# estebandito22/Amplifai-DeepContentRecommenders

Hardware: AMD Instinct MI355X
Metric: training triplets/sec (whole node) + AUC@val, DCUE d=128 at 1/2/4/8 MI355X (higher is better)
Workload: dtype f32 (conv forwards, input and weight gradients: f32 values as power-of-two-scaled split fp16 hi+lo pairs on f16 MFMA, f32 accumulate)

## Files before the change

### amplifai-deepcontentrecommenders_amd/csrc/adam.hip

```cpp
#include <mutex>
#include <unordered_map>

#include "dcue_internal.h"
#include "tgemm.h"
#include "bn0adam.h"


DCUE_KTRACE_READER(adam)

namespace dcue {

__device__ __forceinline__ bool idle_moments(float m, float v) {
  return (__float_as_uint(m) | __float_as_uint(v)) == 0u;
}
__device__ __forceinline__ bool idle_moments4(const float4& m, const float4& v) {
  return (__float_as_uint(m.x) | __float_as_uint(m.y) | __float_as_uint(m.z) | __float_as_uint(m.w) |
          __float_as_uint(v.x) | __float_as_uint(v.y) | __float_as_uint(v.z) | __float_as_uint(v.w)) == 0u;
}
__device__ __forceinline__ float wave_max(float x) {
#pragma unroll
  for (int o = 32; o > 0; o >>= 1) x = fmaxf(x, __shfl_xor(x, o));
  return x;
}
__device__ __forceinline__ float wave_min(float x) {
// ... 718 lines not shown
  sc.one_m_b2 = (float)(1.0 - a->beta2);
  sc.bc2_sqrt = (float)pow(bc2, 0.5);
  sc.eps = (float)a->eps;
  sc.wd = (float)a->weight_decay;
  sc.inv_bc2_sqrt = 1.0f / sc.bc2_sqrt;
  return sc;
}


__global__ __launch_bounds__(256) void k_bn0_grads_adam(const float* __restrict__ G, const float* __restrict__ E,
                                                        const float* gamma0, const float* beta0, const float* mean0,
                                                        const float* invstd0, int H, float* dgamma0, float* dbeta0,
                                                        Bn0AdamDev a) {
  critical_path_priority();
  __shared__ float rg[256], rb[256];
  bn0_channel<true>(G, E, gamma0, beta0, mean0, invstd0, H, dgamma0, dbeta0, a, nullptr, nullptr, nullptr,
                    blockIdx.x, threadIdx.x, rg, rb, true);
}

Bn0AdamDev bn0adam_dev(const Bn0Adam& a) {
  const dcue_model* md = a.md;
  Bn0AdamDev d;
  d.p = md->params; d.m = md->exp_avg; d.v = md->exp_avg_sq; d.g = md->grads;
  d.o_w1 = a.poff[seg_conv_w(1)]; d.o_cb1 = a.poff[seg_conv_b(1)];
  d.o_g0 = a.bn ? a.poff[seg_bn_w(0)] : -1; d.o_b0 = a.bn ? a.poff[seg_bn_b(0)] : -1;
  d.o_g1 = a.bn ? a.poff[seg_bn_w(1)] : -1; d.o_b1 = a.bn ? a.poff[seg_bn_b(1)] : -1;
  d.sc = form_scalars(&a.args);
  d.seg1 = pack_args(md, a.poff).seg[0];
  d.wpack = md->wpack;
  return d;
}

int launch_bn0_grads_adam(const float* G, const float* E, const float* gamma0, const float* beta0,
                          const float* mean0, const float* invstd0, int H, float* dgamma0, float* dbeta0,
                          const Bn0Adam& a, hipStream_t s) {
  const dcue_model* md = a.md;
  if (H > 256) return DCUE_ERR_UNSUPPORTED;
  if (!md->params || !md->grads || !md->exp_avg || !md->exp_avg_sq || a.args.grad_div > 1.0) return DCUE_ERR_INVALID;
  const Bn0AdamDev d = bn0adam_dev(a);
  DCUE_LAUNCH(k_bn0_grads_adam, dim3(kMels), dim3(256), 0, s, G, E, gamma0, beta0, mean0, invstd0, H, dgamma0,
              dbeta0, d);
  DCUE_LAUNCH_CHECK();
  return DCUE_OK;
}

long adam_dense_blocks(long len) { return len >= 512L * 1024 ? 512 : (len / 4 + 255) / 256 + 1; }

int launch_adam(const dcue_model* md, const dcue_adam_args* a, const int64_t* poff, hipStream_t s,
                bool flush_slice, long dense_lo, long dense_hi, bool defer_dgrad2, unsigned* sig) {
  const AdamScalars sc = form_scalars(a);
  const float gdiv = a->grad_div > 1.0 ? (float)a->grad_div : 0.f;
  const int parts = a->parts ? a->parts : (DCUE_ADAM_DENSE | DCUE_ADAM_EMBEDDING);
  const long n = dense_hi >= 0 ? dense_hi : poff[DCUE_N_DENSE_SEGMENTS];
  if (parts & DCUE_ADAM_DENSE) {
    const long len = n - dense_lo;
    const long blocks = adam_dense_blocks(len);
// ... 74 lines not shown
```

### amplifai-deepcontentrecommenders_amd/csrc/bn0adam.h

```cpp
#pragma once

#include "dcue_internal.h"

namespace dcue {

#define DCUE_RHD __device__ __forceinline__
DCUE_RHD float rn_fma(float a, float b, float c) { return __fmaf_rn(a, b, c); }
DCUE_RHD float rn_mul(float a, float b) { return __fmul_rn(a, b); }
DCUE_RHD float rn_add(float a, float b) { return __fadd_rn(a, b); }
DCUE_RHD float rn_sub(float a, float b) { return __fsub_rn(a, b); }
DCUE_RHD float rn_div(float a, float b) { return __fdiv_rn(a, b); }
DCUE_RHD float rn_sqrt(float a) { return __builtin_sqrtf(a); }

}

#include "adam_replay.h"

namespace dcue {

struct Bn0AdamDev {
  float *p, *m, *v, *g;
  long o_w1, o_cb1, o_g0, o_b0, o_g1, o_b1;
  AdamScalars sc;
  PackSeg seg1;
  float* wpack;
};

__device__ __forceinline__ void adam_at(const Bn0AdamDev& a, long idx, float gr) {
  float pp = a.p[idx], mm = a.m[idx], vv = a.v[idx];
  adam_elem(pp, gr, mm, vv, a.sc);
  a.p[idx] = pp;
  a.m[idx] = mm;
  a.v[idx] = vv;
}
Bn0AdamDev bn0adam_dev(const Bn0Adam& a);

template <bool ADAM>
DCUE_RHD void bn0_channel(const float* __restrict__ G, const float* __restrict__ E, const float* gamma0,
                          const float* beta0, const float* mean0, const float* invstd0, int H, float* dgamma0,
                          float* dbeta0, const Bn0AdamDev& a, const float* __restrict__ W1, float* dW1, float* db1,
                          int c, int t, float* rg, float* rb, bool active) {
  float* __restrict__ P = a.p;
  float* __restrict__ Mo = a.m;
  float* __restrict__ V = a.v;
  float* __restrict__ Gd = a.g;
  float dg = 0.f, db = 0.f;
  float pg = 0.f, mg = 0.f, vg = 0.f, pb = 0.f, mb = 0.f, vb = 0.f;
  if (active) {
    if (ADAM && t == 0 && a.o_g0 >= 0) {
      pg = P[a.o_g0 + c]; mg = Mo[a.o_g0 + c]; vg = V[a.o_g0 + c];
      pb = P[a.o_b0 + c]; mb = Mo[a.o_b0 + c]; vb = V[a.o_b0 + c];
    }
    const Bn0Chan ch = bn0_chan(gamma0, beta0, mean0, invstd0, c);
    constexpr int kMaxIt = 4;
#pragma unroll
    for (int it = 0; it < kMaxIt; ++it) {
      const int e = t + 256 * it;
      if (e < 4 * H) {
        const int o = e >> 2, k = e & 3;
        const long wi = ((long)o * kMels + c) * 4 + k;
        if constexpr (ADAM) {
          const long idx = a.o_w1 + wi;
          float pp = P[idx];
          const float gw = bn0_elem(G, E, H, ch, o, k, c, pp, dg, db);
          Gd[idx] = gw;
          float mm = Mo[idx], vv = V[idx];
          adam_elem(pp, gw, mm, vv, a.sc);
          P[idx] = pp;
          Mo[idx] = mm;
          V[idx] = vv;
          pack_store(a.seg1, wi, pp, a.wpack);
        } else {
          dW1[wi] = bn0_elem(G, E, H, ch, o, k, c, W1[wi], dg, db);
        }
      }
    }
    if constexpr (ADAM) {
      if (c == 0)
        for (int o = t; o < H; o += 256) {
          a.g[a.o_cb1 + o] = E[o];
          adam_at(a, a.o_cb1 + o, E[o]);
        }
      if (c == 1 && a.o_g1 >= 0)
        for (int o = t; o < H; o += 256) {
          adam_at(a, a.o_g1 + o, a.g[a.o_g1 + o]);
          adam_at(a, a.o_b1 + o, a.g[a.o_b1 + o]);
        }
    } else {
      if (c == 0)
        for (int o = t; o < H; o += 256) db1[o] = E[o];
    }
  }
  rg[t] = dg;
  rb[t] = db;
  __syncthreads();
  for (int off = 128; off > 0; off >>= 1) {
    if (t < off) {
      rg[t] += rg[t + off];
      rb[t] += rb[t + off];
    }
    __syncthreads();
  }
  if (active && t == 0) {
    dgamma0[c] = rg[0];
    dbeta0[c] = rb[0];
    if (ADAM && a.o_g0 >= 0) {
      adam_elem(pg, rg[0], mg, vg, a.sc);
      adam_elem(pb, rb[0], mb, vb, a.sc);
      P[a.o_g0 + c] = pg; Mo[a.o_g0 + c] = mg; V[a.o_g0 + c] = vg;
      P[a.o_b0 + c] = pb; Mo[a.o_b0 + c] = mb; V[a.o_b0 + c] = vb;
    }
  }
}

}
```

### amplifai-deepcontentrecommenders_amd/csrc/capi.hip

```cpp
#include <math.h>
#include <atomic>
#include <functional>
#include <string.h>

#include "dcue_internal.h"

using namespace dcue;

namespace dcue {

unsigned sync_event_flags() {
  static const unsigned f = [] {
    const char* e = getenv("DCUE_EVENT_SCOPE");
    return (e && e[0] == 's') ? (unsigned)hipEventDisableTiming
                              : (unsigned)(hipEventDisableTiming | hipEventReleaseToDevice);
  }();
  return f;
}

SidePool* side_pool() {
  static SidePool pools[64];
  int dev = 0;
  if (hipGetDevice(&dev) != hipSuccess || dev < 0 || dev >= 64) return nullptr;
  SidePool& p = pools[dev];
// ... 1395 lines not shown
    wa.x_a = l == 1 ? w.invstd[0] : w.a[l - 1];
    wa.x_beta = l == 1 ? nullptr : c.beta_bwd(w, l - 1);
    wa.g_l = w.g[l]; wa.y_l = w.y[l]; wa.idx_l = w.idx[l];
    wa.mean_l = w.mean[l]; wa.invstd_l = w.invstd[l]; wa.a_l = w.a[l];
    wa.dz_acc = bn_acc(w.bnbacc, w.cmax, l); wa.dgamma = c.dgamma(w, l); wa.dbeta = c.dbeta(w, l);
    wa.invN = c.bn ? (float)(1.0 / (copies * gm.lp)) : 0.f;
    wa.bn_world = bn_world;
    wa.counts = w.counts;
    wa.M = M; wa.cout = C; wa.cin = cin;
    wa.wpart = w.wpart[ps]; wa.bpart = w.bpart[ps];
    if (f16w) {
      wa.x_range = rng_at(w, l - 1); wa.y_range = rng_at(w, l); wa.g_range = grng_at(w, l);
      wa.kd_max = kd_max * wa.invN;
    }
    if (l == 1 && inputs_dev) wa.wait = o.inputs_wait;
    const int nch = wgrad_nchunk(l, M, C, cin);
    if (l == 1 && !f16w) {
      TRY(launch_conv1_dx(wa, w.dx1, so));
      wa.g_l = w.dx1;
    }
    TimerScope tsc;
    TRY(timer_begin(&tsc, l == 1 ? DCUE_TIMED_CONV1_WGRAD : -1, so));
    HPROF("capi:19");
    TRY(launch_conv_wgrad(l, l == 1 ? src : SRC_ACT, wa, nch, so));
    HPROF("capi:20");
    TRY(timer_end(&tsc));
    HPROF("capi:21");
    if (l != 1) {
      ForkAfter fk(sp, so, tail);
      TRY(launch_wgrad_reduce(l, wa.wpart, wa.bpart, nch, C, cin, c.Gd(seg_conv_w(l)),
                              c.Gd(seg_conv_b(l)), w.G, w.S, so));
      return fk.done();
    }
    TRY(launch_wgrad_reduce(l, wa.wpart, wa.bpart, nch, C, cin, c.Gd(seg_conv_w(l)),
                            c.Gd(seg_conv_b(l)), w.G, w.S, so));
    ForkAfter fk(sp, so, tail);
    const bool graw = f16w && src == SRC_TRACK_F16;
    if (fuse_late) {
      Bn0Adam ba;
      ba.md = m; ba.poff = c.poff; ba.args = *o.dense_split; ba.bn = c.bn;
      TRY(launch_bn0_grads_adam(w.G, w.S, c.gamma(w, 0), c.beta(w, 0), graw ? w.mean[0] : nullptr,
                                graw ? w.invstd[0] : nullptr, H, c.dgamma(w, 0), c.dbeta(w, 0), ba, so));
      TRY(fk.done());
      if (!probes_on()) return DCUE_OK;
      TRY(probe(PR_G_1, m->grads, late, so));
      return probe(PR_P_EARLY, m->params, late, so);
    }
    TRY(launch_bn0_grads(w.G, w.S, c.P(seg_conv_w(1)), c.gamma(w, 0), c.beta(w, 0),
                         graw ? w.mean[0] : nullptr, graw ? w.invstd[0] : nullptr, H,
                         c.Gd(seg_conv_w(1)), c.dgamma(w, 0), c.dbeta(w, 0),
                         c.Gd(seg_conv_b(1)), so));
    TRY(fk.done());
    return probe(PR_G_1, m->grads, late, so);
  };
  if (ev_x0) TRY(wait_point(s, ev_x0));
  if (o.wait_inputs && !inputs_via_late) {
    TRY(side.wait(o.ahead ? ahead_seq : o.wait_inputs_seq));
    if (!inputs_dev) TRY(wait_point(s, o.wait_inputs));
  }
  TRY(debug_delay(DCUE_SITE_WGRAD_1, s));
  TRY(issue_wgrad(1, s, 2, o.dense_split && !o.comm ? nullptr : &tail[0]));
  HPROF("capi:22");

  if (!thr) {
    if (c.res || c.text) TRY(fc_text_wgrad());
    if (fork_once()) ev_layer[3] = ev_layer[2];
// ... 140 lines not shown
```

### amplifai-deepcontentrecommenders_amd/csrc/conv_wgrad.hip

```cpp
#include "dcue_internal.h"
#include "bn0adam.h"

namespace dcue {

DCUE_KTRACE_READER(wgrad)
static constexpr int kWgradRch = 72;

template <int SRCX, int KS, int PAD, int LIN, int R, int POOL, int LP, int RCH, bool EDGES, bool RAW = false>
__device__ __forceinline__ void wgrad_body(const WgradArgs& a, int bx, int by, int bz, float* lds) {
  constexpr int PW = 128 + 16;
  constexpr int NB = EDGES ? 5 : 1;
  constexpr int FR = RCH / 8;
  constexpr bool TRACK = SRCX == SRC_TRACK_F16 || SRCX == SRC_TRACK_F32;
  float* dzs = lds;
  float* xs = lds + RCH * PW;
  float (*bsum)[NB][128] = reinterpret_cast<float (*)[NB][128]>(lds + 2 * RCH * PW);

  const int tid = threadIdx.x, lane = tid & 63, wave = tid >> 6;
  const int g = lane >> 4, l16 = lane & 15;
  const int wo = wave >> 1, wk = wave & 1;
  const int cout = a.cout, cin = a.cin, kcn = KS * cin;
  const int obase = by * 128, kcbase = bx * 128;
  const long total = (long)a.M * R;
  const long r_begin = (long)bz * a.rows_per_chunk;
// ... 634 lines not shown

constexpr int kW16tO = 64;
constexpr int kW16tThreads = 512;
constexpr int kWgItems = 128;
template <int R, int KS>
constexpr int w16t_img_rows() { return kW16Rows + (KS - 1) * (R >= kW16Rows ? 2 : kW16Rows / R + 2); }
template <int R, int KS>
constexpr size_t w16t_lds_bytes(bool xraw) {
  const size_t st = (size_t)2 * kW16Rows * 128 + (size_t)(xraw ? 1 : 2) * w16t_img_rows<R, KS>() * 256 +
                    (size_t)(kW16tO + 128 + 2 * kWgItems) * sizeof(int);
  const size_t ep = (size_t)kW16tO * (KS * 128 + 4) * sizeof(float);
  return st > ep ? st : ep;
}
__device__ __forceinline__ int w16_off128(int r, int ch) { return 128 * r + 16 * (ch ^ ((r & 2) | ((r >> 1) & 4))); }

template <int SRCX, int KS, int PAD, int LIN, int R, int POOL, int LP>
__device__ __forceinline__ void wgrad16t_body(const WgradArgs& a, int by, int bz, char* lds) {
  constexpr int RCH = kW16Rows;
  constexpr bool TRACK = SRCX == SRC_TRACK_F16 || SRCX == SRC_TRACK_F32;
  constexpr bool EDGES = TRACK;
  constexpr int NB = EDGES ? 5 : 1;
  constexpr int HALO = KS - 1;
  constexpr int IMG = w16t_img_rows<R, KS>();
  constexpr int FX = (IMG + 15) / 16;
  static_assert(KS == 4 && POOL == 4 && R % POOL == 0, "8 waves = 4 taps x 2 o halves; 16 windows per stage");
  constexpr bool TWO = R >= RCH;
  constexpr bool XRAW = SRCX == SRC_TRACK_F16;
  static_assert(TRACK || SRCX == SRC_ACT, "x: the track table (layer 1) or y_{l-1}");
  char* dzh = lds;
  char* dzl = dzh + RCH * 128;
  char* xh = dzl + RCH * 128;
  char* xl = xh + IMG * 256;
  int* exp_o = reinterpret_cast<int*>(xh + (XRAW ? 1 : 2) * IMG * 256);
// ... 280 lines not shown

  DCUE_KT(KID, 3);
  int eo_bias;
  {
    constexpr int KC = KS * 128, PITCH = KC + 4;
    int eo_r[2][4], ec_r[8];
#pragma unroll
    for (int m = 0; m < 2; ++m)
#pragma unroll
      for (int j = 0; j < 4; ++j) eo_r[m][j] = exp_o[32 * oh + 16 * m + 4 * g + j];
#pragma unroll
    for (int n = 0; n < 8; ++n) ec_r[n] = exp_c[16 * n + l16];
    eo_bias = tid < kW16tO ? exp_o[tid] : 0;
    __syncthreads();
    float* tl = reinterpret_cast<float*>(lds);
#pragma unroll
    for (int n = 0; n < 8; ++n)
#pragma unroll
      for (int m = 0; m < 2; ++m)
#pragma unroll
        for (int j = 0; j < 4; ++j)
          tl[(32 * oh + 16 * m + 4 * g + j) * PITCH + kx * 128 + 16 * n + l16] =
              ldexpf(acc[m][n][j], -(eo_r[m][j] + ec_r[n]));
    __syncthreads();
    const int nrow = min(kW16tO, cout - obase);
    float* wp = a.wpart + ((size_t)bz * cout + obase) * KC;
    constexpr int Q = KC / 4;
    for (int i = tid; i < nrow * Q; i += kW16tThreads) {
      const int r = i / Q, k4 = i - r * Q;
      st4(wp + (size_t)r * KC + 4 * k4, *reinterpret_cast<const float4*>(tl + r * PITCH + 4 * k4));
    }
    __syncthreads();
  }
  if (dzt)
#pragma unroll
    for (int e = 0; e < NB; ++e) st4(&bsum[ws][e][4 * q], bacc[e]);
  __syncthreads();
  if (tid < kW16tO && obase + tid < cout) {
#pragma unroll
    for (int e = 0; e < NB; ++e) {
      float v = 0.f;
#pragma unroll
      for (int sl = 0; sl < 16; ++sl) v += bsum[sl][e][tid];
      a.bpart[((size_t)bz * NB + e) * cout + obase + tid] = ldexpf(v, -eo_bias);
    }
  }
  DCUE_KT(KID, 4);
  DCUE_KTW(KID, 7);
}

template <int SRCX, int KS, int PAD, int LIN, int R, int POOL, int LP>
__global__ __launch_bounds__(kW16tThreads, 1) void k_conv_wgrad16t(WgradArgs a) {
  if constexpr (SRCX != SRC_ACT) critical_path_priority();
  extern __shared__ __attribute__((aligned(16))) char lds16t[];
  const int ot = (a.cout + kW16tO - 1) / kW16tO;
  const int L = xcd_swizzle(blockIdx.x, gridDim.x);
  wgrad16t_body<SRCX, KS, PAD, LIN, R, POOL, LP>(a, L % ot, L / ot, lds16t);
  if constexpr (SRCX != SRC_ACT) dev_wait_order(a.wait);
}

constexpr int kW1kO = 32;
constexpr int kW1kThreads = 256;
template <int R, int KS>
constexpr size_t w1k_lds_bytes() {
  const size_t st = (size_t)2 * kW16Rows * 128 + (size_t)w16t_img_rows<R, KS>() * 256 + kW1kO * sizeof(int) +
                    (size_t)kWgItems * (sizeof(int) + sizeof(float));
  const size_t ep = (size_t)kW1kO * (128 + 4) * sizeof(float);
  const size_t bs = (size_t)16 * 5 * kW1kO * sizeof(float);
  const size_t m = st > ep ? st : ep;
  return m > bs ? m : bs;
}

// ... 667 lines not shown
  if (wgrad_f16_on() && !bound)
    n = (rows + w16_rows_per_chunk(rows, (int)n) - 1) / w16_rows_per_chunk(rows, (int)n);
  return (int)(n < 1 ? 1 : n);
}

int wgrad_kernel(int layer, int cin, int cout, int src, bool alone) {
  if (layer == 1) {
    if (!wgrad_f16_on()) return WK_CONV1;
    if (src == SRC_TRACK_F16 && w1k_layer1(cin, cout)) return WK_1K;
    return w16t_layer(1, cin) ? WK_16T : WK_16;
  }
  if (alone && layer == 2 && w16t_layer(2, cin)) return WK_16T;
  return wgrad_f16_on() ? WK_MULTI_F16 : WK_MULTI_F32;
}

void wgrad_shape(int layer, int M, int cout, int cin, int src, bool alone, int32_t* out) {
  const LayerGeom gm = layer_geom(layer == 6 ? 5 : layer);
  const long rows = (long)M * gm.lp * gm.pool;
  const int kernel = wgrad_kernel(layer, cin, cout, src, alone);
  const int nchunk = wgrad_nchunk(layer, M, cout, cin);
  const long rpc = wgrad_chunk_rows(kernel, rows, nchunk);
  out[0] = kernel;
  out[1] = nchunk;
  out[2] = (int32_t)rpc;
  out[3] = (int32_t)(rows - (nchunk - 1) * rpc);
}

template <int L, int SRCX>
static int wgrad_layer(const WgradArgs& a0, int nchunk, hipStream_t s) {
  constexpr LayerGeom gm = layer_geom(L);
// ... 4 lines not shown
  static bool attr = false;
  if (!attr) {
    DCUE_HIP_CHECK(hipFuncSetAttribute((const void*)kern, hipFuncAttributeMaxDynamicSharedMemorySize,
                                       (int)LDS));
    attr = true;
  }
  WgradArgs a = a0;
  const long rows = (long)a.M * R;
  a.rows_per_chunk = (int)wgrad_chunk_rows(WK_F32, rows, nchunk);
  dim3 grid((unsigned)((gm.ks * a.cin + 127) / 128), (unsigned)((a.cout + 127) / 128), (unsigned)nchunk);
  DCUE_LAUNCH(kern, grid, dim3(256), LDS, s, a);
  DCUE_LAUNCH_CHECK();
  return DCUE_OK;
}

template <int L, int SRCX>
static int wgrad16t_launch(const WgradArgs& a0, int nchunk, hipStream_t s) {
  constexpr LayerGeom gm = layer_geom(L);
  constexpr int R = gm.lp * gm.pool;
  constexpr size_t LDS = w16t_lds_bytes<R, gm.ks>(SRCX == SRC_TRACK_F16);
  auto kern = k_conv_wgrad16t<SRCX, gm.ks, gm.pad, gm.lin, R, gm.pool, gm.lp>;
  if (a0.cin != kMels || a0.cout % 4) return DCUE_ERR_INVALID;
  static bool attr = false;
  if (!attr) {
    DCUE_HIP_CHECK(hipFuncSetAttribute((const void*)kern, hipFuncAttributeMaxDynamicSharedMemorySize, (int)LDS));
    attr = true;
  }
  WgradArgs a = a0;
  const long rows = (long)a.M * R;
  if (rows >= (1L << 30)) return DCUE_ERR_UNSUPPORTED;
  a.rows_per_chunk = (int)wgrad_chunk_rows(WK_16T, rows, nchunk);
  if (SRCX != SRC_ACT && R >= kW16Rows && a.rows_per_chunk / R + 3 > kWgItems) return DCUE_ERR_INVALID;
  const unsigned ot = (unsigned)((a.cout + kW16tO - 1) / kW16tO);
  DCUE_LAUNCH(kern, dim3(ot * (unsigned)nchunk), dim3(kW16tThreads), LDS, s, a);
  DCUE_LAUNCH_CHECK();
  return DCUE_OK;
// ... 17 lines not shown
  if (a.rows_per_chunk / R + 3 > kWgItems) return DCUE_ERR_INVALID;
  const unsigned tiles = (unsigned)(((a.cout + kW1kO - 1) / kW1kO) * gm.ks);
  DCUE_LAUNCH(kern, dim3(tiles * (unsigned)nchunk), dim3(kW1kThreads), LDS, s, a);
  DCUE_LAUNCH_CHECK();
  return DCUE_OK;
}

template <int L, int SRCX>
static int wgrad16_layer(const WgradArgs& a0, int nchunk, hipStream_t s) {
  constexpr LayerGeom gm = layer_geom(L);
  constexpr int R = gm.lp * gm.pool;
  if constexpr (L == 1) {
    const int kernel = wgrad_kernel(1, a0.cin, a0.cout, SRCX, true);
    if constexpr (SRCX == SRC_TRACK_F16)
      if (kernel == WK_1K) return wgrad1k_launch(a0, nchunk, s);
    if (kernel == WK_16T) return wgrad16t_launch<1, SRCX>(a0, nchunk, s);
  }
  auto kern = k_conv_wgrad16<SRCX, gm.ks, gm.pad, gm.lin, R, gm.pool, gm.lp, L == 1>;
  static bool attr = false;
  if (!attr) {
    DCUE_HIP_CHECK(hipFuncSetAttribute((const void*)kern, hipFuncAttributeMaxDynamicSharedMemorySize,
                                       (int)kW16LdsB));
    attr = true;
  }
  WgradArgs a = a0;
  const long rows = (long)a.M * R;
  if (rows >= (1L << 30)) return DCUE_ERR_UNSUPPORTED;
  a.rows_per_chunk = (int)wgrad_chunk_rows(WK_16, rows, nchunk);
  dim3 grid((unsigned)((gm.ks * a.cin + 127) / 128), (unsigned)((a.cout + 127) / 128), (unsigned)nchunk);
  DCUE_LAUNCH(kern, grid, dim3(256), kW16LdsB, s, a);
  DCUE_LAUNCH_CHECK();
// ... 10 lines not shown
      case 4: return wgrad16_layer<4, SRC_ACT>(a, nchunk, s);
      case 5: return wgrad16_layer<5, SRC_ACT>(a, nchunk, s);
      default: return DCUE_ERR_INVALID;
    }
  }
  switch (layer) {
    case 1: (void)src; return conv1_wgrad(a, nchunk, s);
    case 2: return wgrad_layer<2, SRC_ACT>(a, nchunk, s);
    case 3: return wgrad_layer<3, SRC_ACT>(a, nchunk, s);
    case 4: return wgrad_layer<4, SRC_ACT>(a, nchunk, s);
    case 5: return wgrad_layer<5, SRC_ACT>(a, nchunk, s);
    default: return DCUE_ERR_INVALID;
  }
}

constexpr int kRedGroups = 8, kRedBatch = 8;

__device__ __forceinline__ float4 sum_chunks(const float* __restrict__ base, size_t stride, int nchunk,
                                             int grp) {
  float4 acc = make_float4(0.f, 0.f, 0.f, 0.f);
  for (int z0 = grp; z0 < nchunk; z0 += kRedGroups * kRedBatch) {
    float4 v[kRedBatch];
#pragma unroll
    for (int i = 0; i < kRedBatch; ++i) {
      const int z = z0 + kRedGroups * i;
      v[i] = z < nchunk ? ld4(base + (size_t)z * stride) : make_float4(0.f, 0.f, 0.f, 0.f);
    }
#pragma unroll
    for (int i = 0; i < kRedBatch; ++i) {
      acc.x += v[i].x; acc.y += v[i].y; acc.z += v[i].z; acc.w += v[i].w;
    }
// ... 125 lines not shown
  const int nb = layer == 1 ? 5 : 1;
  const long nblk = ((long)cout * gm.ks * cin + 127) / 128 + ((long)nb * cout + 127) / 128;
  DCUE_LAUNCH(k_wgrad_reduce, dim3((unsigned)nblk), dim3(256), 0, s, wpart, bpart, nchunk, cout, cin,
                     gm.ks, nb, dW, db, layer == 1 ? G_tmp : nullptr, layer == 1 ? E_tmp : nullptr);
  DCUE_LAUNCH_CHECK();
  return DCUE_OK;
}

__global__ __launch_bounds__(256) void k_bn0_grads(const float* __restrict__ G, const float* __restrict__ E,
                                                   const float* __restrict__ W1, const float* gamma0,
                                                   const float* beta0, const float* mean0,
                                                   const float* invstd0, int H, float* dW1,
                                                   float* dgamma0, float* dbeta0, float* db1) {
  critical_path_priority();
  __shared__ float rg[256], rb[256];
  bn0_channel<false>(G, E, gamma0, beta0, mean0, invstd0, H, dgamma0, dbeta0, Bn0AdamDev{}, W1, dW1, db1,
                     blockIdx.x, threadIdx.x, rg, rb, true);
}

int launch_bn0_grads(const float* G, const float* E, const float* W1, const float* gamma0,
                     const float* beta0, const float* mean0, const float* invstd0, int H, float* dW1,
                     float* dgamma0, float* dbeta0, float* db1, hipStream_t s) {
  DCUE_LAUNCH(k_bn0_grads, dim3(kMels), dim3(256), 0, s, G, E, W1, gamma0, beta0, mean0, invstd0, H, dW1,
              dgamma0, dbeta0, db1);
  DCUE_LAUNCH_CHECK();
  return DCUE_OK;
}

}
```

### amplifai-deepcontentrecommenders_amd/csrc/dcue_internal.h

```cpp
#pragma once

#include <atomic>
#include <vector>

#include <functional>

#include "dcue_common.h"
#include "bnacc.h"

namespace dcue {
bool host_profile_on();
void host_profile_mark(const char* label);
bool on_side_worker();
}
#define HPROF(label)                                          \
  do {                                                        \
    if (::dcue::host_profile_on() && !::dcue::on_side_worker()) ::dcue::host_profile_mark(label); \
  } while (0)

#define TRY(x)                 \
  do {                         \
    int _st = (x);             \
    if (_st) return _st;       \
  } while (0)
// ... 90 lines not shown
  const float* g_l;
  const float* y_l;
  const uint8_t* idx_l;
  const float* mean_l;
  const float* invstd_l;
  const float* a_l;
  const unsigned long long* dz_acc;
  float* dgamma;
  float* dbeta;
  float invN;
  const float* counts;
  int M, cout, cin;
  int rows_per_chunk;
  float* wpart;
  float* bpart;
  const unsigned* x_range;
  const unsigned* y_range;
  const unsigned* g_range;
  float kd_max;
};
__device__ __forceinline__ double bn_grad_scale(const WgradArgs& a) { return a.bn_world > 1 ? 1.0 / a.bn_world : 1.0; }

constexpr int kWgradMultiMax = 5;
struct WgradMulti {
  int n;
  int layer[kWgradMultiMax];
  WgradArgs a[kWgradMultiMax];
  int nchunk[kWgradMultiMax];
  float *dW[kWgradMultiMax], *db[kWgradMultiMax];
  int kt[kWgradMultiMax], ot[kWgradMultiMax];
// ... 35 lines not shown
                        int cin, float* dW, float* db, float* G_tmp, float* E_tmp, hipStream_t s);
struct Bn0Chan {
  float ga, be, m0, i0;
  bool raw;
};
__device__ __forceinline__ Bn0Chan bn0_chan(const float* gamma0, const float* beta0, const float* mean0,
                                            const float* invstd0, int c) {
  Bn0Chan r;
  r.ga = gamma0[c];
  r.be = beta0[c];
  r.raw = mean0 != nullptr;
  r.m0 = r.raw ? mean0[c] : 0.f;
  r.i0 = r.raw ? invstd0[c] : 1.f;
  return r;
}
__device__ __forceinline__ float bn0_elem(const float* __restrict__ G, const float* __restrict__ E, int H,
                                          const Bn0Chan& ch, int o, int k, int c, float w, float& dg, float& db) {
  const float e0 = E[o], e1 = E[H + o], e2 = E[2 * H + o], e3 = E[3 * H + o], e4 = E[4 * H + o];
  const float sv = k == 0 ? (e0 - e1) - e2 : k == 1 ? e0 - e1 : k == 2 ? e0 - e4 : (e0 - e3) - e4;
  const float gr = G[(size_t)o * 4 * kMels + k * kMels + c];
  const float gv = ch.raw ? ch.i0 * fmaf(-ch.m0, sv, gr) : gr;
  dg = fmaf(w, gv, dg);
  db = fmaf(w, sv, db);
  return fmaf(ch.ga, gv, ch.be * sv);
}
constexpr int seg_bn_w(int l) { return l == 0 ? 0 : 4 + 4 * (l - 1); }
constexpr int seg_bn_b(int l) { return l == 0 ? 1 : 5 + 4 * (l - 1); }
constexpr int seg_conv_w(int l) { return 2 + 4 * (l - 1); }
constexpr int seg_conv_b(int l) { return 3 + 4 * (l - 1); }
constexpr int SEG_FC_W = 22, SEG_FC_B = 23, SEG_L1_W = 24, SEG_L1_B = 25, SEG_L2_W = 26, SEG_L2_B = 27;
constexpr int SEG_TX_W = 28, SEG_TX_B = 29;
static_assert(SEG_FC_W == seg_bn_b(5) + 1 && SEG_TX_B + 1 == DCUE_N_DENSE_SEGMENTS, "one index per segment");
static_assert(DCUE_SEG_LATE == seg_conv_w(2), "the late segments are bn0, conv 1 and bn1");
struct AdamScalars;
AdamScalars form_scalars(const dcue_adam_args* a);

struct Bn0Adam {
  const dcue_model* md;
  const int64_t* poff;
  dcue_adam_args args;
  bool bn;
};
int launch_bn0_grads_adam(const float* G, const float* E, const float* gamma0, const float* beta0,
                          const float* mean0, const float* invstd0, int H, float* dgamma0, float* dbeta0,
                          const Bn0Adam& a, hipStream_t s);

int launch_bn0_grads(const float* G, const float* E, const float* W1, const float* gamma0,
                     const float* beta0, const float* mean0, const float* invstd0, int H, float* dW1,
                     float* dgamma0, float* dbeta0, float* db1, hipStream_t s);

int launch_input_stats(int src, const void* tracks, const int32_t* item_track, const float* counts,
                       int M, unsigned long long* acc, unsigned* range, hipStream_t s);
int launch_bn_eval(int C, const float* gamma, const float* rmean, const float* rvar, float* mean,
                   float* invstd, float* a, hipStream_t s);

struct WpackLayout {
  long conv_fwd[6], conv_bwd[6], conv_f16[6], conv_f16b[6];
  long text_f16;
  long total;
};
inline WpackLayout wpack_layout(const dcue_dims* dm) {
  WpackLayout w = {};
  const long H = st_hidden(dm), D = st_feature(dm);
  long n = 0;
// ... 274 lines not shown
```

### profiles/summarize_pmc.py

```python
import csv
import glob
import json
import os
import sys

KERNELS = {"conv1_wgrad": "k_conv1_wgrad", "conv1_wgrad16": "k_conv_wgrad16t<0,", "conv1_wgrad1k": "k_conv_wgrad1k<",
           "wgrad16t_layer2": "k_conv_wgrad16t<2,", "wgrad16_multi": "k_conv_wgrad16_multi", "emb_flush_rows": "k_emb_flush_rows",
           "conv1_fwd": "k_conv_rows<0, 0,", "text_fwd": "k_text_fwd", "user_fwd": "k_user_fwd",
           "text_wgrad": "k_text_wgrad"}
MARK = "spin_kernel"


def _rows(d, pattern):
    rows = []
    for f in glob.glob(os.path.join(d, "**", pattern), recursive=True):
        with open(f) as fh:
            rows += list(csv.DictReader(fh))
    return rows


def _window_by_dispatch(rows):
    ids = sorted({int(r["Dispatch_Id"]) for r in rows if MARK in r.get("Kernel_Name", "")})
    return (ids[0], ids[-1]) if len(ids) >= 2 else None

# ... 81 lines not shown
```

Measured before the change: 6.350 million.

## Fuse layer-1 wgrad partial reduction into BN0 grads/Adam tail kernel

Layer-1 wgrad16t partials are now written channel-major so that each per-mel-channel block of a new tail kernel can reduce its own chunk partials in LDS. That block then feeds the result straight into the BN0 gradient and Adam update, which removes the separate wgrad_reduce launch and the round trip of G/E through global memory. It also prefetches Adam state into registers before the reduction so those loads overlap. The risks are extra LDS use per block, a swizzled transposed store in the wgrad epilogue, and reduction parallelism limited to kMels blocks.

Result: no change. 6.397 million, median of 6 (+0.7%).

```diff
diff --git a/amplifai-deepcontentrecommenders_amd/csrc/adam.hip b/amplifai-deepcontentrecommenders_amd/csrc/adam.hip
--- a/amplifai-deepcontentrecommenders_amd/csrc/adam.hip
+++ b/amplifai-deepcontentrecommenders_amd/csrc/adam.hip
@@ -756,8 +756,21 @@
                                                         Bn0AdamDev a) {
   critical_path_priority();
   __shared__ float rg[256], rb[256];
-  bn0_channel<true>(G, E, gamma0, beta0, mean0, invstd0, H, dgamma0, dbeta0, a, nullptr, nullptr, nullptr,
-                    blockIdx.x, threadIdx.x, rg, rb, true);
+  Bn0Regs r;
+  bn0_load<true>(r, a, nullptr, H, blockIdx.x, threadIdx.x, true);
+  bn0_channel<true>(G, E, gamma0, beta0, mean0, invstd0, H, dgamma0, dbeta0, a, r, nullptr, nullptr, blockIdx.x,
+                    threadIdx.x, rg, rb, true);
+}
+
+__global__ __launch_bounds__(256) void k_w1_tail_adam(const float* __restrict__ wpart1,
+                                                      const float* __restrict__ bpart, int nchunk,
+                                                      const float* gamma0, const float* beta0, const float* mean0,
+                                                      const float* invstd0, int H, float* dgamma0, float* dbeta0,
+                                                      Bn0AdamDev a) {
+  critical_path_priority();
+  __shared__ W1TailLds L;
+  w1_tail_channel<true>(wpart1, bpart, nchunk, gamma0, beta0, mean0, invstd0, H, dgamma0, dbeta0, a, nullptr,
+                        nullptr, nullptr, blockIdx.x, threadIdx.x, L);
 }
 
 Bn0AdamDev bn0adam_dev(const Bn0Adam& a) {
@@ -782,6 +795,19 @@
   const Bn0AdamDev d = bn0adam_dev(a);
   DCUE_LAUNCH(k_bn0_grads_adam, dim3(kMels), dim3(256), 0, s, G, E, gamma0, beta0, mean0, invstd0, H, dgamma0,
               dbeta0, d);
+  DCUE_LAUNCH_CHECK();
+  return DCUE_OK;
+}
+
+int launch_w1_tail_adam(const float* wpart1, const float* bpart, int nchunk, const float* gamma0,
+                        const float* beta0, const float* mean0, const float* invstd0, int H, float* dgamma0,
+                        float* dbeta0, const Bn0Adam& a, hipStream_t s) {
+  const dcue_model* md = a.md;
+  if (H > kTailMaxH || H % 4 || nchunk < 1) return DCUE_ERR_UNSUPPORTED;
+  if (!md->params || !md->grads || !md->exp_avg || !md->exp_avg_sq || a.args.grad_div > 1.0) return DCUE_ERR_INVALID;
+  const Bn0AdamDev d = bn0adam_dev(a);
+  DCUE_LAUNCH(k_w1_tail_adam, dim3(kMels), dim3(256), 0, s, wpart1, bpart, nchunk, gamma0, beta0, mean0, invstd0,
+              H, dgamma0, dbeta0, d);
   DCUE_LAUNCH_CHECK();
   return DCUE_OK;
 }
diff --git a/amplifai-deepcontentrecommenders_amd/csrc/bn0adam.h b/amplifai-deepcontentrecommenders_amd/csrc/bn0adam.h
--- a/amplifai-deepcontentrecommenders_amd/csrc/bn0adam.h
+++ b/amplifai-deepcontentrecommenders_amd/csrc/bn0adam.h
@@ -26,31 +26,66 @@
   float* wpack;
 };
 
-__device__ __forceinline__ void adam_at(const Bn0AdamDev& a, long idx, float gr) {
-  float pp = a.p[idx], mm = a.m[idx], vv = a.v[idx];
+Bn0AdamDev bn0adam_dev(const Bn0Adam& a);
+
+struct Bn0Regs {
+  float pg, mg, vg, pb, mb, vb;
+  float p[4], m[4], v[4];
+  float x[3][3];
+};
+__device__ __forceinline__ void adam_pre(const Bn0AdamDev& a, long idx, float gr, const float (&s)[3]) {
+  float pp = s[0], mm = s[1], vv = s[2];
   adam_elem(pp, gr, mm, vv, a.sc);
   a.p[idx] = pp;
   a.m[idx] = mm;
   a.v[idx] = vv;
 }
-Bn0AdamDev bn0adam_dev(const Bn0Adam& a);
-
 template <bool ADAM>
+DCUE_RHD void bn0_load(Bn0Regs& r, const Bn0AdamDev& a, const float* __restrict__ W1, int H, int c, int t,
+                       bool active) {
+  r.pg = r.mg = r.vg = r.pb = r.mb = r.vb = 0.f;
+  if (ADAM && active && t == 0 && a.o_g0 >= 0) {
+    r.pg = a.p[a.o_g0 + c]; r.mg = a.m[a.o_g0 + c]; r.vg = a.v[a.o_g0 + c];
+    r.pb = a.p[a.o_b0 + c]; r.mb = a.m[a.o_b0 + c]; r.vb = a.v[a.o_b0 + c];
+  }
+#pragma unroll
+  for (int j = 0; j < 3; ++j) r.x[j][0] = r.x[j][1] = r.x[j][2] = 0.f;
+  if (ADAM && active && t < H) {
+    if (c == 0) {
+      r.x[0][0] = a.p[a.o_cb1 + t]; r.x[0][1] = a.m[a.o_cb1 + t]; r.x[0][2] = a.v[a.o_cb1 + t];
+    } else if (c == 1 && a.o_g1 >= 0) {
+      r.x[0][0] = a.p[a.o_g1 + t]; r.x[0][1] = a.m[a.o_g1 + t]; r.x[0][2] = a.v[a.o_g1 + t];
+      r.x[1][0] = a.p[a.o_b1 + t]; r.x[1][1] = a.m[a.o_b1 + t]; r.x[1][2] = a.v[a.o_b1 + t];
+      r.x[2][0] = a.g[a.o_g1 + t]; r.x[2][1] = a.g[a.o_b1 + t];
+    }
+  }
+#pragma unroll
+  for (int it = 0; it < 4; ++it) {
+    const int e = t + 256 * it;
+    r.p[it] = r.m[it] = r.v[it] = 0.f;
+    if (active && e < 4 * H) {
+      const long wi = ((long)(e >> 2) * kMels + c) * 4 + (e & 3);
+      if constexpr (ADAM) {
+        r.p[it] = a.p[a.o_w1 + wi]; r.m[it] = a.m[a.o_w1 + wi]; r.v[it] = a.v[a.o_w1 + wi];
+      } else {
+        r.p[it] = W1[wi];
+      }
+    }
+  }
+}
+
+template <bool ADAM, bool CM = false>
 DCUE_RHD void bn0_channel(const float* __restrict__ G, const float* __restrict__ E, const float* gamma0,
                           const float* beta0, const float* mean0, const float* invstd0, int H, float* dgamma0,
-                          float* dbeta0, const Bn0AdamDev& a, const float* __restrict__ W1, float* dW1, float* db1,
-                          int c, int t, float* rg, float* rb, bool active) {
+                          float* dbeta0, const Bn0AdamDev& a, const Bn0Regs& r, float* dW1, float* db1, int c,
+                          int t, float* rg, float* rb, bool active) {
   float* __restrict__ P = a.p;
   float* __restrict__ Mo = a.m;
   float* __restrict__ V = a.v;
   float* __restrict__ Gd = a.g;
   float dg = 0.f, db = 0.f;
-  float pg = 0.f, mg = 0.f, vg = 0.f, pb = 0.f, mb = 0.f, vb = 0.f;
+  float pg = r.pg, mg = r.mg, vg = r.vg, pb = r.pb, mb = r.mb, vb = r.vb;
   if (active) {
-    if (ADAM && t == 0 && a.o_g0 >= 0) {
-      pg = P[a.o_g0 + c]; mg = Mo[a.o_g0 + c]; vg = V[a.o_g0 + c];
-      pb = P[a.o_b0 + c]; mb = Mo[a.o_b0 + c]; vb = V[a.o_b0 + c];
-    }
     const Bn0Chan ch = bn0_chan(gamma0, beta0, mean0, invstd0, c);
     constexpr int kMaxIt = 4;
 #pragma unroll
@@ -61,31 +96,29 @@
         const long wi = ((long)o * kMels + c) * 4 + k;
         if constexpr (ADAM) {
           const long idx = a.o_w1 + wi;
-          float pp = P[idx];
-          const float gw = bn0_elem(G, E, H, ch, o, k, c, pp, dg, db);
+          float pp = r.p[it];
+          const float gw = bn0_elem<CM>(G, E, H, ch, o, k, c, pp, dg, db);
           Gd[idx] = gw;
-          float mm = Mo[idx], vv = V[idx];
+          float mm = r.m[it], vv = r.v[it];
           adam_elem(pp, gw, mm, vv, a.sc);
           P[idx] = pp;
           Mo[idx] = mm;
           V[idx] = vv;
           pack_store(a.seg1, wi, pp, a.wpack);
         } else {
-          dW1[wi] = bn0_elem(G, E, H, ch, o, k, c, W1[wi], dg, db);
+          dW1[wi] = bn0_elem<CM>(G, E, H, ch, o, k, c, r.p[it], dg, db);
         }
       }
     }
     if constexpr (ADAM) {
-      if (c == 0)
-        for (int o = t; o < H; o += 256) {
-          a.g[a.o_cb1 + o] = E[o];
-          adam_at(a, a.o_cb1 + o, E[o]);
-        }
-      if (c == 1 && a.o_g1 >= 0)
-        for (int o = t; o < H; o += 256) {
-          adam_at(a, a.o_g1 + o, a.g[a.o_g1 + o]);
-          adam_at(a, a.o_b1 + o, a.g[a.o_b1 + o]);
-        }
+      if (c == 0 && t < H) {
+        a.g[a.o_cb1 + t] = E[t];
+        adam_pre(a, a.o_cb1 + t, E[t], r.x[0]);
+      }
+      if (c == 1 && a.o_g1 >= 0 && t < H) {
+        adam_pre(a, a.o_g1 + t, r.x[2][0], r.x[0]);
+        adam_pre(a, a.o_b1 + t, r.x[2][1], r.x[1]);
+      }
     } else {
       if (c == 0)
         for (int o = t; o < H; o += 256) db1[o] = E[o];
@@ -113,4 +146,74 @@
   }
 }
 
-}
+constexpr int kRedGroups = 8, kRedBatch = 8;
+constexpr int kTailMaxH = 128;
+constexpr int kTailCols = kTailMaxH + 5 * kTailMaxH / 4;
+struct W1TailLds {
+  float4 red[kRedGroups][kTailCols];
+  float G[4 * kTailMaxH], E[5 * kTailMaxH];
+  float rg[256], rb[256];
+};
+
+template <bool ADAM>
+DCUE_RHD void w1_tail_channel(const float* __restrict__ wpart1, const float* __restrict__ bpart, int nchunk,
+                              const float* gamma0, const float* beta0, const float* mean0, const float* invstd0,
+                              int H, float* dgamma0, float* dbeta0, const Bn0AdamDev& a,
+                              const float* __restrict__ W1, float* dW1, float* db1, int c, int t, W1TailLds& L) {
+  Bn0Regs r;
+  bn0_load<ADAM>(r, a, W1, H, c, t, true);
+  const int ncol = H + 5 * H / 4;
+  const int npair = kRedGroups * ncol;
+  const size_t gstride = (size_t)kMels * 4 * H, estride = (size_t)5 * H;
+  const float* gbase = wpart1 + (size_t)c * 4 * H;
+  constexpr int NP = 9, NS = 5;
+  for (int p0 = t; p0 < npair; p0 += 256 * NP) {
+    const float* base[NP];
+    size_t stride[NP];
+    int grp[NP], col[NP];
+    float4 acc[NP];
+#pragma unroll
+    for (int q = 0; q < NP; ++q) {
+      const int p = min(p0 + 256 * q, npair - 1);
+      grp[q] = p / ncol;
+      col[q] = p - grp[q] * ncol;
+      const bool isg = col[q] < H;
+      base[q] = isg ? gbase + 4 * col[q] : bpart + 4 * (col[q] - H);
+      stride[q] = isg ? gstride : estride;
+      acc[q] = make_float4(0.f, 0.f, 0.f, 0.f);
+    }
+    for (int zb = 0; zb < nchunk; zb += kRedGroups * NS) {
+      float4 v[NP][NS];
+#pragma unroll
+      for (int q = 0; q < NP; ++q)
+#pragma unroll
+        for (int i = 0; i < NS; ++i) {
+          const int z = zb + grp[q] + kRedGroups * i;
+          v[q][i] = z < nchunk ? ld4(base[q] + (size_t)z * stride[q]) : make_float4(0.f, 0.f, 0.f, 0.f);
+        }
+#pragma unroll
+      for (int q = 0; q < NP; ++q)
+#pragma unroll
+        for (int i = 0; i < NS; ++i) {
+          acc[q].x += v[q][i].x; acc[q].y += v[q][i].y; acc[q].z += v[q][i].z; acc[q].w += v[q][i].w;
+        }
+    }
+#pragma unroll
+    for (int q = 0; q < NP; ++q)
+      if (p0 + 256 * q < npair) L.red[grp[q]][col[q]] = acc[q];
+  }
+  __syncthreads();
+  for (int cl = t; cl < ncol; cl += 256) {
+    float4 s = L.red[0][cl];
+#pragma unroll
+    for (int g = 1; g < kRedGroups; ++g) {
+      s.x += L.red[g][cl].x; s.y += L.red[g][cl].y; s.z += L.red[g][cl].z; s.w += L.red[g][cl].w;
+    }
+    *reinterpret_cast<float4*>(cl < H ? L.G + 4 * cl : L.E + 4 * (cl - H)) = s;
+  }
+  __syncthreads();
+  bn0_channel<ADAM, true>(L.G, L.E, gamma0, beta0, mean0, invstd0, H, dgamma0, dbeta0, a, r, dW1, db1, c, t,
+                          L.rg, L.rb, true);
+}
+
+}
diff --git a/amplifai-deepcontentrecommenders_amd/csrc/capi.hip b/amplifai-deepcontentrecommenders_amd/csrc/capi.hip
--- a/amplifai-deepcontentrecommenders_amd/csrc/capi.hip
+++ b/amplifai-deepcontentrecommenders_amd/csrc/capi.hip
@@ -1433,6 +1433,8 @@
       wa.kd_max = kd_max * wa.invN;
     }
     if (l == 1 && inputs_dev) wa.wait = o.inputs_wait;
+    const bool tail1 = l == 1 && w1_tail_fused(cin, C, src);
+    wa.wpart_cmajor = tail1;
     const int nch = wgrad_nchunk(l, M, C, cin);
     if (l == 1 && !f16w) {
       TRY(launch_conv1_dx(wa, w.dx1, so));
@@ -1451,24 +1453,33 @@
                               c.Gd(seg_conv_b(l)), w.G, w.S, so));
       return fk.done();
     }
-    TRY(launch_wgrad_reduce(l, wa.wpart, wa.bpart, nch, C, cin, c.Gd(seg_conv_w(l)),
-                            c.Gd(seg_conv_b(l)), w.G, w.S, so));
+    if (!tail1)
+      TRY(launch_wgrad_reduce(l, wa.wpart, wa.bpart, nch, C, cin, c.Gd(seg_conv_w(l)),
+                              c.Gd(seg_conv_b(l)), w.G, w.S, so));
     ForkAfter fk(sp, so, tail);
     const bool graw = f16w && src == SRC_TRACK_F16;
+    const float* mean0 = graw ? w.mean[0] : nullptr;
+    const float* invstd0 = graw ? w.invstd[0] : nullptr;
     if (fuse_late) {
       Bn0Adam ba;
       ba.md = m; ba.poff = c.poff; ba.args = *o.dense_split; ba.bn = c.bn;
-      TRY(launch_bn0_grads_adam(w.G, w.S, c.gamma(w, 0), c.beta(w, 0), graw ? w.mean[0] : nullptr,
-                                graw ? w.invstd[0] : nullptr, H, c.dgamma(w, 0), c.dbeta(w, 0), ba, so));
+      if (tail1)
+        TRY(launch_w1_tail_adam(wa.wpart, wa.bpart, nch, c.gamma(w, 0), c.beta(w, 0), mean0, invstd0, H,
+                                c.dgamma(w, 0), c.dbeta(w, 0), ba, so));
+      else
+        TRY(launch_bn0_grads_adam(w.G, w.S, c.gamma(w, 0), c.beta(w, 0), mean0, invstd0, H, c.dgamma(w, 0),
+                                  c.dbeta(w, 0), ba, so));
       TRY(fk.done());
       if (!probes_on()) return DCUE_OK;
       TRY(probe(PR_G_1, m->grads, late, so));
       return probe(PR_P_EARLY, m->params, late, so);
     }
-    TRY(launch_bn0_grads(w.G, w.S, c.P(seg_conv_w(1)), c.gamma(w, 0), c.beta(w, 0),
-                         graw ? w.mean[0] : nullptr, graw ? w.invstd[0] : nullptr, H,
-                         c.Gd(seg_conv_w(1)), c.dgamma(w, 0), c.dbeta(w, 0),
-                         c.Gd(seg_conv_b(1)), so));
+    if (tail1)
+      TRY(launch_w1_tail(wa.wpart, wa.bpart, nch, c.P(seg_conv_w(1)), c.gamma(w, 0), c.beta(w, 0), mean0, invstd0,
+                         H, c.Gd(seg_conv_w(1)), c.dgamma(w, 0), c.dbeta(w, 0), c.Gd(seg_conv_b(1)), so));
+    else
+      TRY(launch_bn0_grads(w.G, w.S, c.P(seg_conv_w(1)), c.gamma(w, 0), c.beta(w, 0), mean0, invstd0, H,
+                           c.Gd(seg_conv_w(1)), c.dgamma(w, 0), c.dbeta(w, 0), c.Gd(seg_conv_b(1)), so));
     TRY(fk.done());
     return probe(PR_G_1, m->grads, late, so);
   };
diff --git a/amplifai-deepcontentrecommenders_amd/csrc/conv_wgrad.hip b/amplifai-deepcontentrecommenders_amd/csrc/conv_wgrad.hip
--- a/amplifai-deepcontentrecommenders_amd/csrc/conv_wgrad.hip
+++ b/amplifai-deepcontentrecommenders_amd/csrc/conv_wgrad.hip
@@ -672,9 +672,10 @@
 }
 __device__ __forceinline__ int w16_off128(int r, int ch) { return 128 * r + 16 * (ch ^ ((r & 2) | ((r >> 1) & 4))); }
 
-template <int SRCX, int KS, int PAD, int LIN, int R, int POOL, int LP>
+template <int SRCX, int KS, int PAD, int LIN, int R, int POOL, int LP, bool CMAJ = false>
 __device__ __forceinline__ void wgrad16t_body(const WgradArgs& a, int by, int bz, char* lds) {
   constexpr int RCH = kW16Rows;
+  static_assert(!CMAJ || SRCX != SRC_ACT, "channel-major partials: layer 1 (the fused tail reads them)");
   constexpr bool TRACK = SRCX == SRC_TRACK_F16 || SRCX == SRC_TRACK_F32;
   constexpr bool EDGES = TRACK;
   constexpr int NB = EDGES ? 5 : 1;
@@ -985,21 +986,44 @@
     eo_bias = tid < kW16tO ? exp_o[tid] : 0;
     __syncthreads();
     float* tl = reinterpret_cast<float*>(lds);
-#pragma unroll
-    for (int n = 0; n < 8; ++n)
-#pragma unroll
-      for (int m = 0; m < 2; ++m)
-#pragma unroll
-        for (int j = 0; j < 4; ++j)
-          tl[(32 * oh + 16 * m + 4 * g + j) * PITCH + kx * 128 + 16 * n + l16] =
-              ldexpf(acc[m][n][j], -(eo_r[m][j] + ec_r[n]));
-    __syncthreads();
     const int nrow = min(kW16tO, cout - obase);
-    float* wp = a.wpart + ((size_t)bz * cout + obase) * KC;
-    constexpr int Q = KC / 4;
-    for (int i = tid; i < nrow * Q; i += kW16tThreads) {
-      const int r = i / Q, k4 = i - r * Q;
-      st4(wp + (size_t)r * KC + 4 * k4, *reinterpret_cast<const float4*>(tl + r * PITCH + 4 * k4));
+    if constexpr (CMAJ) {
+      constexpr int PL = 128 * kW16tO;
+#pragma unroll
+      for (int n = 0; n < 8; ++n) {
+        const int cc = 16 * n + l16;
+        const int sw = (cc & 3) | ((cc & 12) << 1);
+#pragma unroll
+        for (int m = 0; m < 2; ++m)
+#pragma unroll
+          for (int j = 0; j < 4; ++j)
+            tl[kx * PL + cc * kW16tO + ((32 * oh + 16 * m + 4 * g + j) ^ sw)] =
+                ldexpf(acc[m][n][j], -(eo_r[m][j] + ec_r[n]));
+      }
+      __syncthreads();
+      float* wp = a.wpart + ((size_t)bz * 128 * cout + obase) * KS;
+      for (int i = tid; i < PL; i += kW16tThreads) {
+        const int cc = i / kW16tO, ol = i % kW16tO;
+        const int off = cc * kW16tO + (ol ^ ((cc & 3) | ((cc & 12) << 1)));
+        if (ol < nrow)
+          st4(wp + ((size_t)cc * cout + ol) * KS, make_float4(tl[off], tl[PL + off], tl[2 * PL + off], tl[3 * PL + off]));
+      }
+    } else {
+#pragma unroll
+      for (int n = 0; n < 8; ++n)
+#pragma unroll
+        for (int m = 0; m < 2; ++m)
+#pragma unroll
+          for (int j = 0; j < 4; ++j)
+            tl[(32 * oh + 16 * m + 4 * g + j) * PITCH + kx * 128 + 16 * n + l16] =
+                ldexpf(acc[m][n][j], -(eo_r[m][j] + ec_r[n]));
+      __syncthreads();
+      float* wp = a.wpart + ((size_t)bz * cout + obase) * KC;
+      constexpr int Q = KC / 4;
+      for (int i = tid; i < nrow * Q; i += kW16tThreads) {
+        const int r = i / Q, k4 = i - r * Q;
+        st4(wp + (size_t)r * KC + 4 * k4, *reinterpret_cast<const float4*>(tl + r * PITCH + 4 * k4));
+      }
     }
     __syncthreads();
   }
@@ -1020,13 +1044,13 @@
   DCUE_KTW(KID, 7);
 }
 
-template <int SRCX, int KS, int PAD, int LIN, int R, int POOL, int LP>
+template <int SRCX, int KS, int PAD, int LIN, int R, int POOL, int LP, bool CMAJ = false>
 __global__ __launch_bounds__(kW16tThreads, 1) void k_conv_wgrad16t(WgradArgs a) {
   if constexpr (SRCX != SRC_ACT) critical_path_priority();
   extern __shared__ __attribute__((aligned(16))) char lds16t[];
   const int ot = (a.cout + kW16tO - 1) / kW16tO;
   const int L = xcd_swizzle(blockIdx.x, gridDim.x);
-  wgrad16t_body<SRCX, KS, PAD, LIN, R, POOL, LP>(a, L % ot, L / ot, lds16t);
+  wgrad16t_body<SRCX, KS, PAD, LIN, R, POOL, LP, CMAJ>(a, L % ot, L / ot, lds16t);
   if constexpr (SRCX != SRC_ACT) dev_wait_order(a.wait);
 }
 
@@ -1724,6 +1748,14 @@
   return wgrad_f16_on() ? WK_MULTI_F16 : WK_MULTI_F32;
 }
 
+bool w1_tail_fused(int cin, int cout, int src) {
+  static const bool on = [] {
+    const char* e = getenv("DCUE_W1_TAIL");
+    return !(e && e[0] == 's');
+  }();
+  return on && cout <= kTailMaxH && cout % 4 == 0 && wgrad_kernel(1, cin, cout, src, true) == WK_16T;
+}
+
 void wgrad_shape(int layer, int M, int cout, int cin, int src, bool alone, int32_t* out) {
   const LayerGeom gm = layer_geom(layer == 6 ? 5 : layer);
   const long rows = (long)M * gm.lp * gm.pool;
@@ -1758,12 +1790,12 @@
   return DCUE_OK;
 }
 
-template <int L, int SRCX>
+template <int L, int SRCX, bool CMAJ = false>
 static int wgrad16t_launch(const WgradArgs& a0, int nchunk, hipStream_t s) {
   constexpr LayerGeom gm = layer_geom(L);
   constexpr int R = gm.lp * gm.pool;
   constexpr size_t LDS = w16t_lds_bytes<R, gm.ks>(SRCX == SRC_TRACK_F16);
-  auto kern = k_conv_wgrad16t<SRCX, gm.ks, gm.pad, gm.lin, R, gm.pool, gm.lp>;
+  auto kern = k_conv_wgrad16t<SRCX, gm.ks, gm.pad, gm.lin, R, gm.pool, gm.lp, CMAJ>;
   if (a0.cin != kMels || a0.cout % 4) return DCUE_ERR_INVALID;
   static bool attr = false;
   if (!attr) {
@@ -1811,7 +1843,8 @@
     const int kernel = wgrad_kernel(1, a0.cin, a0.cout, SRCX, true);
     if constexpr (SRCX == SRC_TRACK_F16)
       if (kernel == WK_1K) return wgrad1k_launch(a0, nchunk, s);
-    if (kernel == WK_16T) return wgrad16t_launch<1, SRCX>(a0, nchunk, s);
+    if (kernel == WK_16T)
+      return a0.wpart_cmajor ? wgrad16t_launch<1, SRCX, true>(a0, nchunk, s) : wgrad16t_launch<1, SRCX>(a0, nchunk, s);
   }
   auto kern = k_conv_wgrad16<SRCX, gm.ks, gm.pad, gm.lin, R, gm.pool, gm.lp, L == 1>;
   static bool attr = false;
@@ -1852,7 +1885,6 @@
   }
 }
 
-constexpr int kRedGroups = 8, kRedBatch = 8;
 
 __device__ __forceinline__ float4 sum_chunks(const float* __restrict__ base, size_t stride, int nchunk,
                                              int grp) {
@@ -2008,8 +2040,30 @@
                                                    float* dgamma0, float* dbeta0, float* db1) {
   critical_path_priority();
   __shared__ float rg[256], rb[256];
-  bn0_channel<false>(G, E, gamma0, beta0, mean0, invstd0, H, dgamma0, dbeta0, Bn0AdamDev{}, W1, dW1, db1,
+  Bn0Regs r;
+  bn0_load<false>(r, Bn0AdamDev{}, W1, H, blockIdx.x, threadIdx.x, true);
+  bn0_channel<false>(G, E, gamma0, beta0, mean0, invstd0, H, dgamma0, dbeta0, Bn0AdamDev{}, r, dW1, db1,
                      blockIdx.x, threadIdx.x, rg, rb, true);
+}
+
+__global__ __launch_bounds__(256) void k_w1_tail(const float* __restrict__ wpart1, const float* __restrict__ bpart,
+                                                 int nchunk, const float* __restrict__ W1, const float* gamma0,
+                                                 const float* beta0, const float* mean0, const float* invstd0,
+                                                 int H, float* dW1, float* dgamma0, float* dbeta0, float* db1) {
+  critical_path_priority();
+  __shared__ W1TailLds L;
+  w1_tail_channel<false>(wpart1, bpart, nchunk, gamma0, beta0, mean0, invstd0, H, dgamma0, dbeta0, Bn0AdamDev{},
+                         W1, dW1, db1, blockIdx.x, threadIdx.x, L);
+}
+
+int launch_w1_tail(const float* wpart1, const float* bpart, int nchunk, const float* W1, const float* gamma0,
+                   const float* beta0, const float* mean0, const float* invstd0, int H, float* dW1,
+                   float* dgamma0, float* dbeta0, float* db1, hipStream_t s) {
+  if (H > kTailMaxH || H % 4 || nchunk < 1) return DCUE_ERR_UNSUPPORTED;
+  DCUE_LAUNCH(k_w1_tail, dim3(kMels), dim3(256), 0, s, wpart1, bpart, nchunk, W1, gamma0, beta0, mean0, invstd0,
+              H, dW1, dgamma0, dbeta0, db1);
+  DCUE_LAUNCH_CHECK();
+  return DCUE_OK;
 }
 
 int launch_bn0_grads(const float* G, const float* E, const float* W1, const float* gamma0,
diff --git a/amplifai-deepcontentrecommenders_amd/csrc/dcue_internal.h b/amplifai-deepcontentrecommenders_amd/csrc/dcue_internal.h
--- a/amplifai-deepcontentrecommenders_amd/csrc/dcue_internal.h
+++ b/amplifai-deepcontentrecommenders_amd/csrc/dcue_internal.h
@@ -128,6 +128,7 @@
   int rows_per_chunk;
   float* wpart;
   float* bpart;
+  bool wpart_cmajor;
   const unsigned* x_range;
   const unsigned* y_range;
   const unsigned* g_range;
@@ -193,11 +194,12 @@
   r.i0 = r.raw ? invstd0[c] : 1.f;
   return r;
 }
+template <bool CM = false>
 __device__ __forceinline__ float bn0_elem(const float* __restrict__ G, const float* __restrict__ E, int H,
                                           const Bn0Chan& ch, int o, int k, int c, float w, float& dg, float& db) {
   const float e0 = E[o], e1 = E[H + o], e2 = E[2 * H + o], e3 = E[3 * H + o], e4 = E[4 * H + o];
   const float sv = k == 0 ? (e0 - e1) - e2 : k == 1 ? e0 - e1 : k == 2 ? e0 - e4 : (e0 - e3) - e4;
-  const float gr = G[(size_t)o * 4 * kMels + k * kMels + c];
+  const float gr = CM ? G[o * 4 + k] : G[(size_t)o * 4 * kMels + k * kMels + c];
   const float gv = ch.raw ? ch.i0 * fmaf(-ch.m0, sv, gr) : gr;
   dg = fmaf(w, gv, dg);
   db = fmaf(w, sv, db);
@@ -227,6 +229,14 @@
 int launch_bn0_grads(const float* G, const float* E, const float* W1, const float* gamma0,
                      const float* beta0, const float* mean0, const float* invstd0, int H, float* dW1,
                      float* dgamma0, float* dbeta0, float* db1, hipStream_t s);
+
+bool w1_tail_fused(int cin, int cout, int src);
+int launch_w1_tail(const float* wpart1, const float* bpart, int nchunk, const float* W1, const float* gamma0,
+                   const float* beta0, const float* mean0, const float* invstd0, int H, float* dW1,
+                   float* dgamma0, float* dbeta0, float* db1, hipStream_t s);
+int launch_w1_tail_adam(const float* wpart1, const float* bpart, int nchunk, const float* gamma0,
+                        const float* beta0, const float* mean0, const float* invstd0, int H, float* dgamma0,
+                        float* dbeta0, const Bn0Adam& a, hipStream_t s);
 
 int launch_input_stats(int src, const void* tracks, const int32_t* item_track, const float* counts,
                        int M, unsigned long long* acc, unsigned* range, hipStream_t s);
diff --git a/profiles/summarize_pmc.py b/profiles/summarize_pmc.py
--- a/profiles/summarize_pmc.py
+++ b/profiles/summarize_pmc.py
@@ -7,7 +7,8 @@
 KERNELS = {"conv1_wgrad": "k_conv1_wgrad", "conv1_wgrad16": "k_conv_wgrad16t<0,", "conv1_wgrad1k": "k_conv_wgrad1k<",
            "wgrad16t_layer2": "k_conv_wgrad16t<2,", "wgrad16_multi": "k_conv_wgrad16_multi", "emb_flush_rows": "k_emb_flush_rows",
            "conv1_fwd": "k_conv_rows<0, 0,", "text_fwd": "k_text_fwd", "user_fwd": "k_user_fwd",
-           "text_wgrad": "k_text_wgrad"}
+           "text_wgrad": "k_text_wgrad",
+           "w1_tail": "k_w1_tail", "wgrad_reduce": "k_wgrad_reduce(", "bn0_grads": "k_bn0_grads"}
 MARK = "spin_kernel"
 
 
```
